# dvrp0/Monsoon

Measured on NVIDIA B200. Metric: env_steps_per_sec, higher is better.
Workload: dtype u8

## Files before the change

### monsoon_b200/csrc/sbw_core.cuh

```cuda
#pragma once
#include "sb_defs.h"
#include "sbw_warp.cuh"

#define WEF_OWNER 1
#define WEF_STRUCT 2
#define WEF_FIXED 4
#define WEF_SINGLE 8
#define WEF_RPLAY 16
#define WEF_ONB 32

struct __align__(8) WCard { u8 card; i8 cost; u8 flags; i8 link; u16 wn; i16 xstr; };
struct __align__(8) WMem { i8 b005; u8 pos, card, fl; i16 strength; u8 st[5]; i8 parent; u8 pad[4]; };
struct WPly {
  i16 base, max_mana, mana;
  i8 front_line;
  u8 replacable, leftmost, n_hand, n_deck, faction;
  u8 pad[4];
  WCard hand[8];
  WCard deck[24];
};
struct __align__(16) WG {
  i16 e_str[MAXE];
  i16 e_dmg[MAXE];
  u32 e_st[MAXE];
  u8 e_card[MAXE], e_fl[MAXE], e_pos[MAXE], e_mid[MAXE], e_plen[MAXE];
  __align__(8) u8 e_path[MAXE][MAXPATH];
  __align__(8) i8 board[24];
  WPly pl[2];
  u32 seed_lo, seed_hi;
  u32 occ, own1, strc;
  u16 turn, draw, steps;
  u8 local_order, current_order, phase, err, done;
  i8 player_sign;
  u8 hist_n, hist_card[4], hist_owner[4];
  u8 n_ent, n_trig, resolving, depth, n_mem, n_obj, maybe_badobs;
  u8 trig[MAXTRIG];
  __align__(8) WMem mem[NMEM];
  u32 lm[SB_MASK_WORDS];
  i8 scr[24];
  i8 tn_ids[24];
  u8 remap[MAXE];
  __align__(8) double scr_d[DECK_W];
  double feat[SB_N_FEATURES];
  const DCard* cards;
  const double* wt;
};

#define WERR(wg, code) do { if (!(wg)->err) (wg)->err = (code); } while (0)
SBW_FI const DCard& WCARD(const WG* wg, int card) { const DCard* c = wg->cards; W_SHARED(c); return c[card]; }
SBW_FI int wpt_x(int pt) { return pt >= 20 ? -1 : (pt & 3); }
SBW_FI int wpt_y(int pt) { return pt == PT_BASE_REMOTE ? -1 : pt == PT_BASE_LOCAL ? 5 : (pt >> 2); }
SBW_FI bool w_valid_xy(int x, int y) { return (unsigned)x <= 3u && (unsigned)y <= 4u; }
SBW_FI int w_owner(const WG* wg, int id) { return wg->e_fl[id] & WEF_OWNER; }
SBW_FI bool w_is_struct(const WG* wg, int id) { return (wg->e_fl[id] & WEF_STRUCT) != 0; }
SBW_FI int w_st(const WG* wg, int id, int s) { return (int)((wg->e_st[id] >> (SB_ST_BITS * s)) & 63u); }
SBW_FI int w_ex(const WG* wg, int id) { return wg->e_pos[id] & 3; }
SBW_FI int w_ey(const WG* wg, int id) { return wg->e_pos[id] >> 2; }

SBW_FI void w_philox(u32 c0, u32 c1, u32 c2, u32 c3, u32 k0, u32 k1, u32& o0, u32& o1) {
#pragma unroll
  for (int r = 0; r < 10; r++) {
    u32 h0 = w_mulhi(0xD2511F53u, c0), l0 = 0xD2511F53u * c0;
    u32 h1 = w_mulhi(0xCD9E8D57u, c2), l1 = 0xCD9E8D57u * c2;
    u32 n0 = h1 ^ c1 ^ k0, n2 = h0 ^ c3 ^ k1;
    c0 = n0; c1 = l1; c2 = n2; c3 = l0;
    k0 += 0x9E3779B9u; k1 += 0xBB67AE85u;
  }
  o0 = c0; o1 = c1;
}
SBW_NI int w_rng_below(WG* wg, int n) {
  W_SHARED(wg);
  if (n <= 0) { WERR(wg, SB_ERR_EMPTY_CHOICE); return 0; }
  u32 w0, w1;
  w_philox(wg->draw, wg->turn, 0, 0, wg->seed_lo, wg->seed_hi, w0, w1);
  wg->draw++;
  return (int)w_mulhi(w0, (u32)n);
}
SBW_NI double w_rng_random(WG* wg) {
  W_SHARED(wg);
  u32 w0, w1;
  w_philox(wg->draw, wg->turn, 0, 0, wg->seed_lo, wg->seed_hi, w0, w1);
  wg->draw++;
  return d_mul(d_add(d_mul((double)(w0 >> 5), 67108864.0), (double)(w1 >> 6)), 0x1.0p-53);
}
SBW_FI u32 w_agent_pick(u32 seed_lo, u32 seed_hi, u32 step, u32 n) {
  u32 w0, w1;
  w_philox(step, 0, 0xA6E7u, 0, seed_lo, seed_hi, w0, w1);
  return w_mulhi(w0, n);
}
SBW void w_shuffle(WG* wg, i8* a, int n) {
#pragma unroll 1
  for (int i = n - 1; i > 0; i--) {
    int j = w_rng_below(wg, i + 1);
    i8 t = a[i]; a[i] = a[j]; a[j] = t;
  }
}

SBW_FI int w_opponent_of(const WG* wg, int order) { return order == 0 ? 1 - wg->local_order : wg->local_order; }
SBW_FI int w_at_xy(const WG* wg, int x, int y) { return w_valid_xy(x, y) ? wg->board[y * 4 + x] : -1; }
SBW_FI int w_at_pt(const WG* wg, int pt) { return (unsigned)pt < 20u ? wg->board[pt] : -1; }
SBW_FI void w_set_xy(WG* wg, int x, int y, int id) {
  const int t = y * 4 + x;
  const u32 b = 1u << t;
  const int prev = wg->board[t];
  if (prev >= 0 && prev != id) wg->e_fl[prev] &= (u8)~WEF_ONB;
  wg->board[t] = (i8)id;
  if (id >= 0) {
    const u8 fl = wg->e_fl[id] | WEF_ONB;
    wg->e_fl[id] = fl;
    wg->e_pos[id] = (u8)t;
    wg->occ |= b;
    wg->own1 = (fl & WEF_OWNER) ? (wg->own1 | b) : (wg->own1 & ~b);
    wg->strc = (fl & WEF_STRUCT) ? (wg->strc | b) : (wg->strc & ~b);
  } else {
    wg->occ &= ~b;
  }
}
SBW_FI void w_clear_at(WG* wg, int id) {
  const int t = wg->e_pos[id];
  const int victim = wg->board[t];
  if (victim >= 0) wg->e_fl[victim] &= (u8)~WEF_ONB;
  wg->board[t] = -1;
  wg->occ &= ~(1u << t);
}
SBW_FI int w_next_tile(u32& m, bool ascending) {
  int t = ascending ? w_ffs(m) - 1 : 31 - w_clz(m);
  m &= ~(1u << t);
  return t;
}
SBW_FI void w_calc_front_line(WG* wg, int order) {
  const bool local = order == wg->local_order;
// ... 270 lines not shown
  if (!w_is_struct(wg, id)) {
    wg->e_plen[id] = 0;
    if (WCARD(wg, wg->e_card[id]).trigger == TR_ON_DEATH) { w_push_trigger(wg, id, has_source); w_pop_trigger(wg); }
  }
  w_calc_front_line(wg, w_opponent_of(wg, wg->current_order));
}
SBW_NI int w_deal_damage(WG* wg, int id, int amount, int pending, int has_source) {
  W_SHARED(wg);
  const int s0 = wg->e_str[id];
  if (s0 - amount < 0) amount = s0;
  wg->e_dmg[id] = (i16)amount;
  const int s1 = s0 - amount;
  wg->e_str[id] = (i16)s1;
  if (!pending && s1 <= 0) w_destroy(wg, id, has_source);
  else if (!w_is_struct(wg, id) && s1 > 0 && WCARD(wg, wg->e_card[id]).trigger == TR_AFTER_SURVIVING) {
    w_push_trigger(wg, id, has_source);
    w_pop_trigger(wg);
  }
  return amount;
}
SBW_FI int w_deal_damage_pt(WG* wg, int pt, int amount, int has_source) {
  if (pt == PT_BASE_LOCAL) return w_player_damage(wg, wg->local_order, amount);
  if (pt == PT_BASE_REMOTE) return w_player_damage(wg, 1 - wg->local_order, amount);
  int id = w_at_pt(wg, pt);
  if (id < 0) { WERR(wg, SB_ERR_NONE_TARGET); return 0; }
  return w_deal_damage(wg, id, amount, 0, has_source);
}

SBW_FI u8 w_enc_xy(int x, int y) { return (u8)((y + 1) * 4 + x); }
SBW_NI void w_set_path(WG* wg, int id, int on_play, int extra_movement) {
  W_SHARED(wg);
  u64 dest = 0;
  int nd = 0;
  int px = w_ex(wg, id), py = w_ey(wg, id);
  int confused_cached = w_st(wg, id, SB_ST_CONFUSED);
  const int fl = wg->e_fl[id];
  const int owner = fl & WEF_OWNER;
  const bool is_local = owner == wg->local_order;
  int steps = on_play ? WCARD(wg, wg->e_card[id]).movement + extra_movement : 1;
  if (steps > MAXPATH) { WERR(wg, SB_ERR_OVERFLOW); steps = MAXPATH; }
  const u32 mine = owner ? wg->own1 : ~wg->own1;
#pragma unroll 1
  for (int i = 0; i < steps; i++) {
    int dx = px, dy = py + (is_local ? -1 : 1);
    if (confused_cached > 0) {
      int delta;
      if (px == 0) { w_rng_below(wg, 1); delta = 1; }
      else if (px == 3) { w_rng_below(wg, 1); delta = -1; }
      else delta = w_rng_below(wg, 2) == 0 ? -1 : 1;
      dx = px + delta; dy = py;
      confused_cached--;
    } else if (on_play && !(fl & WEF_FIXED) && dy != (is_local ? -1 : 5)) {
      const u32 occ = wg->occ;
      const bool ahead_free_or_own = !w_valid_xy(dx, dy) || !((occ >> (dy * 4 + dx)) & 1u) || ((mine >> (dy * 4 + dx)) & 1u);
      if (ahead_free_or_own) {
        const int t = py * 4 + px;
        bool left_ok = px > 0 && w_valid_xy(px - 1, py) && ((occ & ~mine) >> (t - 1) & 1u);
        bool right_ok = px < 3 && w_valid_xy(px + 1, py) && ((occ & ~mine) >> (t + 1) & 1u);
        const u8 lenc = w_enc_xy(px - 1, py), renc = w_enc_xy(px + 1, py);
#pragma unroll 1
        for (int k = 0; k < nd; k++) {
          const u8 d = (u8)(dest >> (8 * k));
          if (d == lenc) left_ok = false;
          if (d == renc) right_ok = false;
        }
        if (px <= 1) { if (right_ok) { dx = px + 1; dy = py; } else if (left_ok) { dx = px - 1; dy = py; } }
        else { if (left_ok) { dx = px - 1; dy = py; } else if (right_ok) { dx = px + 1; dy = py; } }
      }
    }
    dest |= (u64)w_enc_xy(dx, dy) << (8 * nd);
    nd++;
    px = dx; py = dy;
  }
  *reinterpret_cast<u64*>(wg->e_path[id]) = dest;
  wg->e_plen[id] = (u8)nd;
}
SBW_FI void w_set_path_step(WG* wg, int id) {
  if (w_st(wg, id, SB_ST_CONFUSED)) { w_set_path(wg, id, 0, 0); return; }
  const int t = wg->e_pos[id];
  const bool is_local = w_owner(wg, id) == wg->local_order;
  wg->e_path[id][0] = (u8)(t + 4 + (is_local ? -4 : 4));
  wg->e_plen[id] = 1;
}
SBW_NI void w_unit_move(WG* wg, int id) {
  W_SHARED(wg);
  if (wg->depth > MAXDEPTH) { WERR(wg, SB_ERR_DEPTH); return; }
  wg->depth++;
  const int trig = WCARD(wg, wg->e_card[id]).trigger;
  const u8 current_id = (u8)(wg->e_mid[id] + 1);
  wg->e_mid[id] = current_id;
  if (wg->phase == PH_TURN_START) {
    if (w_st(wg, id, SB_ST_POISONED)) w_deal_damage(wg, id, 1, 0, 0);
    else if (w_st(wg, id, SB_ST_VITALIZED)) wv_heal(wg, id, 1);
    if (w_st(wg, id, SB_ST_FROZEN)) { w_st_remove(wg, id, SB_ST_FROZEN); wg->depth--; return; }
  }
  if (wg->e_plen[id] == 0) { wg->depth--; return; }
  if (trig == TR_BEFORE_MOVING && !w_st(wg, id, SB_ST_DISABLED)) w_ability(wg, id, PT_NONE, 1);
  if (w_st(wg, id, SB_ST_FROZEN)) { wg->depth--; return; }
  const int np = wg->e_plen[id];
  const u64 path = *reinterpret_cast<const u64*>(wg->e_path[id]);
#pragma unroll 1
  for (int i = 0; i < np; i++) {
    const int enc = (int)((path >> (8 * i)) & 0xFFu);
    const int dx = enc & 3, dy = (enc >> 2) - 1;
    const int owner = w_owner(wg, id);
    if (dy < 0 || dy > 4) {
      if (trig == TR_BEFORE_ATTACKING && !w_st(wg, id, SB_ST_DISABLED)) w_ability(wg, id, -2, 1);
      const int target = dy < 0 ? 1 - wg->local_order : wg->local_order;
      w_player_damage(wg, target, wg->e_str[id]);
      if (wg->pl[target].base > 0) w_destroy(wg, id, 0);
      wg->depth--;
      return;
    }
    int tid = w_at_xy(wg, dx, dy);
    bool attacked = false;
    if (tid >= 0 && w_owner(wg, tid) == owner && dx == w_ex(wg, id)) { wg->depth--; return; }
    if (tid >= 0 && (w_st(wg, id, SB_ST_CONFUSED) || w_owner(wg, tid) != owner)) {
      if (trig == TR_BEFORE_ATTACKING && !w_st(wg, id, SB_ST_DISABLED)) w_ability(wg, id, dy * 4 + dx, 1);
      tid = w_at_xy(wg, dx, dy);
      if (tid >= 0) {
        const int tstr = wg->e_str[tid];
        const int t_pending = !w_is_struct(wg, tid) && WCARD(wg, wg->e_card[tid]).trigger == TR_ON_DEATH && !w_st(wg, tid, SB_ST_DISABLED);
        const int l_pending = trig == TR_ON_DEATH && !w_st(wg, id, SB_ST_DISABLED);
        w_deal_damage(wg, tid, wg->e_str[id], t_pending, 0);
        w_deal_damage(wg, id, tstr, l_pending, 0);
        if (wg->e_str[tid] <= 0 && t_pending) w_destroy(wg, tid, 0);
        if (wg->e_str[id] <= 0 && l_pending) w_destroy(wg, id, 0);
        attacked = true;
      }
    }
    if (current_id != wg->e_mid[id]) { wg->depth--; return; }
    if (w_at_xy(wg, dx, dy) < 0 && wg->e_str[id] > 0) {
      w_clear_at(wg, id);
      w_set_xy(wg, dx, dy, id);
      WPly& p = wg->pl[w_owner(wg, id)];
      if (p.front_line > dy) p.front_line = (i8)(dy > 1 ? dy : 1);
      if (attacked && trig == TR_AFTER_ATTACKING && !w_st(wg, id, SB_ST_DISABLED)) w_ability(wg, id, PT_NONE, 1);
      if (w_st(wg, id, SB_ST_CONFUSED)) w_st_remove(wg, id, SB_ST_CONFUSED);
    }
  }
  wg->depth--;
}
SBW_FI void w_unit_play(WG* wg, int id, int x, int y) {
  wg->e_fl[id] |= WEF_RPLAY;
  w_set_xy(wg, x, y, id);
  w_set_path(wg, id, 1, 0);
  if (WCARD(wg, wg->e_card[id]).trigger == TR_ON_PLAY) w_ability(wg, id, PT_NONE, 1);
  w_unit_move(wg, id);
  wg->e_fl[id] &= (u8)~WEF_RPLAY;
}
SBW_NI void w_struct_play(WG* wg, int id, int x, int y) {
  W_SHARED(wg);
  w_set_xy(wg, x, y, id);
  if (WCARD(wg, wg->e_card[id]).trigger == TR_ON_PLAY) w_ability(wg, id, PT_NONE, 1);
}
SBW_FI void w_gain_speed(WG* wg, int id, int amount) { w_set_path(wg, id, (wg->e_fl[id] & WEF_RPLAY) != 0, amount); }
SBW_NI void wv_command(WG* wg, int id) {
  W_SHARED(wg);
  const u8 cache = wg->e_fl[id] & WEF_FIXED;
  wg->e_fl[id] |= WEF_FIXED;
  w_set_path_step(wg, id);
  w_unit_move(wg, id);
  wg->e_fl[id] = (u8)((wg->e_fl[id] & ~WEF_FIXED) | cache);
}
SBW_NI void wv_convert(WG* wg, int id) {
  W_SHARED(wg);
  const int o = w_opponent_of(wg, w_owner(wg, id));
  wg->e_fl[id] = (u8)((wg->e_fl[id] & ~WEF_OWNER) | (o ? WEF_OWNER : 0));
  const int t = wg->e_pos[id];
  if (wg->board[t] == id) {
    const u32 b = 1u << t;
    wg->own1 = o ? (wg->own1 | b) : (wg->own1 & ~b);
  }
  w_set_path(wg, id, (wg->e_fl[id] & WEF_RPLAY) != 0, 0);
}
SBW_NI void wv_push(WG* wg, int id, int fx, int fy) {
  W_SHARED(wg);
  int dx = 0, dy = 0;
  const int ex = w_ex(wg, id), ey = w_ey(wg, id);
  if (fy < ey) dy = 1; else if (fy > ey) dy = -1; else if (fx < ex) dx = 1; else if (fx > ex) dx = -1;
  if (dx || dy) {
#pragma unroll 1
    for (;;) {
      const int nx = w_ex(wg, id) + dx, ny = w_ey(wg, id) + dy;
      if (!w_valid_xy(nx, ny)) break;
      if (wg->board[ny * 4 + nx] >= 0) return;
      w_clear_at(wg, id);
      w_set_xy(wg, nx, ny, id);
    }
  }
  WPly& p = wg->pl[w_owner(wg, id)];
  const int y = w_ey(wg, id);
  if (p.front_line > y) p.front_line = (i8)(y > 1 ? y : 1);
}
SBW_NI void wv_force_attack(WG* wg, int id, int tx, int ty) {
  W_SHARED(wg);
  const int ex = w_ex(wg, id), ey = w_ey(wg, id);
  if ((tx != ex && ty != ey) || w_at_xy(wg, tx, ty) < 0) return;
  u64 dest = 0;
  int nd = 0;
  const bool vertical = (tx == ex);
  const int fixed = vertical ? ex : ey, start = vertical ? ey : ex, end = vertical ? ty : tx;
  const int delta = end > start ? 1 : -1;
#pragma unroll 1
  for (int i = start + delta; i != end + delta; i += delta) {
    const int x = vertical ? fixed : i, y = vertical ? i : fixed;
    if (i != end && w_at_xy(wg, x, y) >= 0) return;
    dest |= (u64)w_enc_xy(x, y) << (8 * nd);
    nd++;
  }
  if (nd > 0) {
    *reinterpret_cast<u64*>(wg->e_path[id]) = dest;
    wg->e_plen[id] = (u8)nd;
    w_unit_move(wg, id);
  }
}
SBW_NI void wv_teleport(WG* wg, int id, int dx, int dy) {
  W_SHARED(wg);
  if (w_at_xy(wg, dx, dy) < 0) {
    w_clear_at(wg, id);
    w_set_xy(wg, dx, dy, id);
    WPly& p = wg->pl[w_owner(wg, id)];
    if (p.front_line > dy) p.front_line = (i8)(dy > 1 ? dy : 1);
    w_set_path(wg, id, (wg->e_fl[id] & WEF_RPLAY) != 0, 0);
  }
// ... 342 lines not shown
```

### monsoon_b200/csrc/sbw_kernels.cu

```cuda
#include <cuda_runtime.h>
#include <stdint.h>
#include <stdlib.h>
#include "sbw_agent.cuh"
#include "sbw_launch.h"

#define W_SLOT_BYTES ((int)((sizeof(WG) + sizeof(SbState) + 15) & ~15u))

__device__ __forceinline__ void kw_stage_cards(DCard* s_cards, const DCard* cards) {
  const u32* src = reinterpret_cast<const u32*>(cards);
  u32* dst = reinterpret_cast<u32*>(s_cards);
  for (int i = threadIdx.x; i < (int)(SBC_COUNT * sizeof(DCard) / 4); i += blockDim.x) dst[i] = __ldg(src + i);
  __syncthreads();
}
__device__ __forceinline__ WG* kw_slot(unsigned char* dyn, int warp, int slot_bytes) { return reinterpret_cast<WG*>(dyn + (size_t)warp * slot_bytes); }
__device__ __forceinline__ SbState* kw_image(WG* wg) { return reinterpret_cast<SbState*>(reinterpret_cast<unsigned char*>(wg) + sizeof(WG)); }
__device__ __forceinline__ void kw_load_record(SbState* img, const u8* states, int gi) {
  const int lane = threadIdx.x & 31;
  reinterpret_cast<uint4*>(img)[lane] = __ldg(reinterpret_cast<const uint4*>(states + (size_t)gi * SB_STATE_BYTES) + lane);
  __syncwarp();
}
__device__ __forceinline__ void kw_store_record(u8* states, int gi, const SbState* img) {
  const int lane = threadIdx.x & 31;
  __syncwarp();
  reinterpret_cast<uint4*>(states + (size_t)gi * SB_STATE_BYTES)[lane] = reinterpret_cast<const uint4*>(img)[lane];
}
__device__ __forceinline__ int kw_next_game(int* queue, int fallback) {
  if (!queue) return fallback;
  int gi = 0;
  if ((threadIdx.x & 31) == 0) gi = atomicAdd(queue, 1);
  return __shfl_sync(0xFFFFFFFFu, gi, 0);
}

template <int WPC, int MINB, int SYNC>
__global__ void __launch_bounds__(WPC * 32, MINB) kw_rollout_random(int n, u8* states, int max_steps, int* steps_out, unsigned long long* chain,
                                                                     const DCard* cards, const double* wt, int* queue) {
  __shared__ DCard s_cards[SBC_COUNT];
  extern __shared__ __align__(16) unsigned char s_dyn[];
  kw_stage_cards(s_cards, cards);
  const int warp = threadIdx.x >> 5, lane = threadIdx.x & 31;
  WG* wg = kw_slot(s_dyn, warp, W_SLOT_BYTES);
  SbState* img = kw_image(wg);
  wg->cards = s_cards; wg->wt = wt;
  const bool digest = chain != nullptr;
  int gi = blockIdx.x * WPC + warp;
  if (SYNC == 0) {
#pragma unroll 1
    for (;;) {
      gi = kw_next_game(queue, gi);
      if (gi >= n) break;
      kw_load_record(img, states, gi);
      w_unpack(wg, img);
      unsigned long long ch = digest ? chain[gi] : 0ull;
      int k = 0;
      bool alive = !(wg->done & SB_DONE) && !wg->err && max_steps > 0;
#pragma unroll 1
      while (alive) {
        w_game_step(wg, w_pick_action(wg));
        w_end_of_step(wg);
        if (digest) { w_pack(wg, img); __syncwarp(); ch = (ch ^ w_digest_state(img)) * 0x100000001B3ull; }
        k++;
        alive = !(wg->done & SB_DONE) && !wg->err && k < max_steps;
      }
      w_pack(wg, img);
      kw_store_record(states, gi, img);
      if (lane == 0) {
        if (steps_out) steps_out[gi] = k;
        if (digest) chain[gi] = ch;
      }
      if (!queue) break;
      __syncwarp();
    }
  } else {
    bool has_game = false, alive = false, at_pass = false, dry = false;
    unsigned long long ch = 0ull;
    int k = 0;
    bool first = true;
#pragma unroll 1
    for (;;) {
      if (!alive && !dry) {
        if (has_game) {
          w_pack(wg, img);
          kw_store_record(states, gi, img);
          if (lane == 0) { if (steps_out) steps_out[gi] = k; if (digest) chain[gi] = ch; }
          __syncwarp();
          has_game = false;
        }
        if (queue) gi = kw_next_game(queue, gi); else if (!first) gi = n;
        first = false;
        if (gi < n) {
          has_game = true;
          kw_load_record(img, states, gi);
          w_unpack(wg, img);
          ch = digest ? chain[gi] : 0ull;
          k = 0; at_pass = false;
          alive = !(wg->done & SB_DONE) && !wg->err && max_steps > 0;
        } else dry = true;
      }
      if (!__syncthreads_or(alive)) break;
#pragma unroll 1
      for (;;) {
        int a = -1;
        if (alive && !at_pass) {
          a = w_pick_action(wg);
          if (a == SB_ACTION_PASS) { at_pass = true; a = -1; }
        }
        if (SYNC == 2) {
          if (a < 0) { __syncthreads(); break; }
        } else if (!__syncthreads_or(a >= 0)) break;
        if (a >= 0) {
          w_game_step(wg, a);
          w_end_of_step(wg);
          if (digest) { w_pack(wg, img); __syncwarp(); ch = (ch ^ w_digest_state(img)) * 0x100000001B3ull; }
          k++;
          alive = !(wg->done & SB_DONE) && !wg->err && k < max_steps;
        }
      }
      if (alive && at_pass) {
        w_game_step(wg, SB_ACTION_PASS);
        w_end_of_step(wg);
        if (digest) { w_pack(wg, img); __syncwarp(); ch = (ch ^ w_digest_state(img)) * 0x100000001B3ull; }
        k++;
        at_pass = false;
        alive = !(wg->done & SB_DONE) && !wg->err && k < max_steps;
      }
    }
    if (has_game) {
      w_pack(wg, img);
      kw_store_record(states, gi, img);
      if (lane == 0) { if (steps_out) steps_out[gi] = k; if (digest) chain[gi] = ch; }
    }
  }
}

template <int WPC>
__global__ void __launch_bounds__(WPC * 32) kw_step(int n, u8* states, const u8* actions, i8* reward, u8* done, u8* err, u32* next_masks,
                                                    const DCard* cards, const double* wt) {
  __shared__ DCard s_cards[SBC_COUNT];
  extern __shared__ __align__(16) unsigned char s_dyn[];
  kw_stage_cards(s_cards, cards);
  const int warp = threadIdx.x >> 5, lane = threadIdx.x & 31;
  WG* wg = kw_slot(s_dyn, warp, W_SLOT_BYTES);
  SbState* img = kw_image(wg);
  wg->cards = s_cards; wg->wt = wt;
#pragma unroll 1
  for (int gi = blockIdx.x * WPC + warp; gi < n; gi += gridDim.x * WPC) {
    kw_load_record(img, states, gi);
    w_unpack(wg, img);
    w_game_step(wg, actions[gi]);
    w_pack(wg, img);
    kw_store_record(states, gi, img);
    if (lane == 0) {
      if (reward) reward[gi] = (wg->done & SB_REWARD) ? 1 : 0;
      if (done) done[gi] = (wg->done & SB_DONE) ? 1 : 0;
      if (err) err[gi] = img->err;
    }
    if (next_masks) {
      w_legal_mask(wg);
      if (lane < SB_MASK_WORDS) next_masks[(size_t)gi * SB_MASK_WORDS + lane] = wg->lm[lane];
    }
    __syncwarp();
  }
}

template <int WPC, int MODE>
__global__ void __launch_bounds__(WPC * 32, 2048 / (WPC * 32)) kw_stream(int n, const u8* states, void* out, u8* err, const DCard* cards) {
  __shared__ DCard s_cards[SBC_COUNT];
  __shared__ __align__(16) SbState s_img[WPC];
  __shared__ __align__(16) int s_out[MODE == 1 ? WPC * SB_OBS_INTS : (MODE == 2 ? WPC * 2 * SB_N_FEATURES : 4)];
  kw_stage_cards(s_cards, cards);
  const int warp = threadIdx.x >> 5, lane = threadIdx.x & 31;
  const int stride = gridDim.x * WPC;
  int gi = blockIdx.x * WPC + warp;
  uint4 nxt = make_uint4(0, 0, 0, 0);
  if (gi < n) nxt = __ldg(reinterpret_cast<const uint4*>(states + (size_t)gi * SB_STATE_BYTES) + lane);
#pragma unroll 1
  for (; gi < n; gi += stride) {
    const uint4 cur = nxt;
    if (gi + stride < n) nxt = __ldg(reinterpret_cast<const uint4*>(states + (size_t)(gi + stride) * SB_STATE_BYTES) + lane);
    reinterpret_cast<uint4*>(&s_img[warp])[lane] = cur;
    __syncwarp();
    if (MODE == 0) {
      u32 m[SB_MASK_WORDS];
      w_legal_mask_packed(&s_img[warp], s_cards, m);
      const u32 v = lane == 0 ? m[0] : lane == 1 ? m[1] : lane == 2 ? m[2] : lane == 3 ? m[3] : m[4];
      if (lane < SB_MASK_WORDS) reinterpret_cast<u32*>(out)[(size_t)gi * SB_MASK_WORDS + lane] = v;
    } else if (MODE == 1) {
      int* ob = s_out + warp * SB_OBS_INTS;
      const int e = w_observe_packed(&s_img[warp], s_cards, ob);
      uint4* dst = reinterpret_cast<uint4*>(reinterpret_cast<int*>(out) + (size_t)gi * SB_OBS_INTS);
      const uint4* src = reinterpret_cast<const uint4*>(ob);
#pragma unroll
      for (int i = lane; i < SB_OBS_INTS / 4; i += 32) dst[i] = src[i];
      if (err && lane == 0) err[gi] = (u8)e;
    } else {
      double* f = reinterpret_cast<double*>(s_out) + warp * SB_N_FEATURES;
      const int e = w_features_packed(&s_img[warp], s_cards, f);
      __syncwarp();
      if (lane < SB_N_FEATURES) reinterpret_cast<double*>(out)[(size_t)gi * SB_N_FEATURES + lane] = f[lane];
      if (err && lane == 0) err[gi] = (u8)e;
    }
    __syncwarp();
  }
}

template <int WPC, int MODE>
__global__ void __launch_bounds__(WPC * 32) kw_query(int n, u8* states, void* out, u8* err, const DCard* cards, const double* wt) {
  __shared__ DCard s_cards[SBC_COUNT];
  extern __shared__ __align__(16) unsigned char s_dyn[];
  kw_stage_cards(s_cards, cards);
  const int warp = threadIdx.x >> 5, lane = threadIdx.x & 31;
  WG* wg = kw_slot(s_dyn, warp, W_SLOT_BYTES);
  SbState* img = kw_image(wg);
  wg->cards = s_cards; wg->wt = wt;
#pragma unroll 1
  for (int gi = blockIdx.x * WPC + warp; gi < n; gi += gridDim.x * WPC) {
    kw_load_record(img, states, gi);
    w_unpack(wg, img);
    if (MODE == 0) {
      w_legal_mask(wg);
      if (lane < SB_MASK_WORDS) reinterpret_cast<u32*>(out)[(size_t)gi * SB_MASK_WORDS + lane] = wg->lm[lane];
    } else if (MODE == 1) {
      const int e = w_observe(wg, reinterpret_cast<int*>(out) + (size_t)gi * SB_OBS_INTS);
      if (err && lane == 0) err[gi] = (u8)e;
    } else if (MODE == 2) {
      w_scan_badobs(wg);
      const int e = w_features(wg, wg->feat);
      if (lane < SB_N_FEATURES) reinterpret_cast<double*>(out)[(size_t)gi * SB_N_FEATURES + lane] = wg->feat[lane];
      if (err && lane == 0) err[gi] = (u8)e;
    } else {
      const int a = w_expert_action(wg);
      if (lane == 0) {
        reinterpret_cast<u8*>(out)[gi] = (u8)a;
        SbState* rec = reinterpret_cast<SbState*>(states + (size_t)gi * SB_STATE_BYTES);
        rec->draw = wg->draw;
        rec->err = wg->err;
      }
    }
    __syncwarp();
  }
}

#define W_HSLOT_BYTES ((int)((2 * sizeof(WG) + sizeof(SbState) + 2 * SB_N_FEATURES * sizeof(double) + 15) & ~15u))
__device__ __forceinline__ WG* kw_hfork(WG* base) { return base + 1; }
__device__ __forceinline__ SbState* kw_himage(WG* base) { return reinterpret_cast<SbState*>(base + 2); }
__device__ __forceinline__ double* kw_hweights(WG* base) { return reinterpret_cast<double*>(reinterpret_cast<unsigned char*>(base + 2) + sizeof(SbState)); }

template <int WPC>
__global__ void __launch_bounds__(WPC * 32) kw_select_action(int n, const u8* states, const double* weights, u8* actions, double* scores,
                                                             const DCard* cards, const double* wt) {
  __shared__ DCard s_cards[SBC_COUNT];
  extern __shared__ __align__(16) unsigned char s_dyn[];
  kw_stage_cards(s_cards, cards);
  const int warp = threadIdx.x >> 5, lane = threadIdx.x & 31;
  WG* base = kw_slot(s_dyn, warp, W_HSLOT_BYTES);
  WG* work = kw_hfork(base);
  SbState* img = kw_himage(base);
  double* w = kw_hweights(base);
  base->cards = s_cards; base->wt = wt; work->cards = s_cards; work->wt = wt;
#pragma unroll 1
  for (int gi = blockIdx.x * WPC + warp; gi < n; gi += gridDim.x * WPC) {
    kw_load_record(img, states, gi);
    w_unpack(base, img);
    w_scan_badobs(base);
    if (lane < SB_N_FEATURES) w[lane] = weights[(size_t)gi * SB_N_FEATURES + lane];
    if (scores) for (int a = lane; a < SB_N_ACTIONS; a += 32) scores[(size_t)gi * SB_N_ACTIONS + a] = __longlong_as_double(0x7FF8000000000000ll);
    __syncwarp();
    const int a = w_decide(base, work, w, scores ? scores + (size_t)gi * SB_N_ACTIONS : nullptr, false);
    if (lane == 0) actions[gi] = (u8)a;
    __syncwarp();
  }
}

template <int WPC, int MINB>
__global__ void __launch_bounds__(WPC * 32, MINB) kw_rollout_heuristic(int n, u8* states, const double* w_first, const double* w_second, const int* idx_first,
                                                                        const int* idx_second, int max_steps, i8* result, int* steps_out,
                                                                        const DCard* cards, const double* wt, int* queue) {
  __shared__ DCard s_cards[SBC_COUNT];
  extern __shared__ __align__(16) unsigned char s_dyn[];
  kw_stage_cards(s_cards, cards);
  const int warp = threadIdx.x >> 5, lane = threadIdx.x & 31;
  WG* base = kw_slot(s_dyn, warp, W_HSLOT_BYTES);
  WG* work = kw_hfork(base);
  SbState* img = kw_himage(base);
  double* wf = kw_hweights(base);
  double* ws = wf + SB_N_FEATURES;
  base->cards = s_cards; base->wt = wt; work->cards = s_cards; work->wt = wt;
  int gi = blockIdx.x * WPC + warp;
#pragma unroll 1
  for (;;) {
    gi = kw_next_game(queue, gi);
    if (gi >= n) break;
    kw_load_record(img, states, gi);
    w_unpack(base, img);
    w_scan_badobs(base);
    if (lane < SB_N_FEATURES) {
      if (w_first) wf[lane] = w_first[(size_t)(idx_first ? idx_first[gi] : gi) * SB_N_FEATURES + lane];
      if (w_second) ws[lane] = w_second[(size_t)(idx_second ? idx_second[gi] : gi) * SB_N_FEATURES + lane];
    }
    __syncwarp();
    int k = 0, res = -1;
#pragma unroll 1
    for (;;) {
      if (k >= max_steps || base->pl[0].base < 0 || base->pl[1].base < 0) break;
      const bool first_to_move = base->player_sign == 1;
      if (first_to_move ? w_first != nullptr : w_second != nullptr) w_decide(base, work, first_to_move ? wf : ws, nullptr, true);
      else {
        const int a = w_expert_action(base);
        w_game_step(base, a);
        w_end_of_step(base);
      }
      k++;
      if (base->err) { res = -2; break; }
    }
    if (res != -2) {
      const bool l0 = base->pl[0].base < 0, l1 = base->pl[1].base < 0;
      res = (l1 && !l0) ? 0 : (l0 && !l1) ? 1 : -1;
    }
    w_pack(base, img);
    kw_store_record(states, gi, img);
    if (lane == 0) {
      if (result) result[gi] = (i8)res;
      if (steps_out) steps_out[gi] = k;
    }
    if (!queue) break;
    __syncwarp();
  }
}

static inline int grid_for(int n, int per) { return (n + per - 1) / per; }
static int g_carveout = -1;
template <class K> static cudaError_t set_smem(K kernel, int bytes) {
  cudaError_t e = cudaFuncSetAttribute(kernel, cudaFuncAttributeMaxDynamicSharedMemorySize, bytes);
  if (e != cudaSuccess || g_carveout < 0) return e;
  return cudaFuncSetAttribute(kernel, cudaFuncAttributePreferredSharedMemoryCarveout, g_carveout);
}
#define W_TRY(x) do { cudaError_t e_ = (x); if (e_ != cudaSuccess) return e_; } while (0)

int sbw_wg_bytes(void) { return (int)sizeof(WG); }

cudaError_t sbw_init(void) {
  { const char* e = getenv("SBW_CARVEOUT"); if (e) g_carveout = atoi(e); }
  W_TRY((set_smem(kw_rollout_random<4, 8, 0>, 4 * W_SLOT_BYTES)));
  W_TRY((set_smem(kw_rollout_random<8, 4, 0>, 8 * W_SLOT_BYTES)));
  W_TRY((set_smem(kw_rollout_random<8, 8, 0>, 8 * W_SLOT_BYTES)));
  W_TRY((set_smem(kw_rollout_random<8, 4, 1>, 8 * W_SLOT_BYTES)));
  W_TRY((set_smem(kw_rollout_random<16, 2, 1>, 16 * W_SLOT_BYTES)));
  W_TRY((set_smem(kw_rollout_random<32, 1, 1>, 32 * W_SLOT_BYTES)));
  W_TRY((set_smem(kw_rollout_random<32, 2, 1>, 32 * W_SLOT_BYTES)));
  W_TRY((set_smem(kw_rollout_random<28, 1, 1>, 28 * W_SLOT_BYTES)));
  W_TRY((set_smem(kw_rollout_random<14, 2, 1>, 14 * W_SLOT_BYTES)));
  W_TRY((set_smem(kw_rollout_random<32, 1, 2>, 32 * W_SLOT_BYTES)));
  W_TRY((set_smem(kw_rollout_random<16, 2, 2>, 16 * W_SLOT_BYTES)));
  W_TRY(set_smem(kw_step<8>, 8 * W_SLOT_BYTES));
  W_TRY(set_smem(kw_query<8, 3>, 8 * W_SLOT_BYTES));
  W_TRY(set_smem(kw_select_action<4>, 4 * W_HSLOT_BYTES));
  W_TRY(set_smem(kw_rollout_heuristic<4, 8>, 4 * W_HSLOT_BYTES));
  W_TRY(set_smem(kw_rollout_heuristic<4, 9>, 4 * W_HSLOT_BYTES));
  return cudaSuccess;
}

void sbw_rollout_random(const SbwCtx* c, int n, uint8_t* states, int max_steps, int32_t* steps, uint64_t* chain, int shape, int grid_override,
                        cudaStream_t st) {
  static const int WPCS[11] = {8, 4, 8, 8, 16, 32, 32, 28, 14, 32, 16}, PER_SM[11] = {4, 8, 8, 4, 2, 1, 2, 1, 2, 1, 2};
  if (shape < 0 || shape > 10) shape = 0;
  const int wpc = WPCS[shape], per_sm = PER_SM[shape];
  const int resident = c->sm_count * per_sm;
  const int full = grid_for(n, wpc);
  int* q = nullptr;
  int grid = full;
  if (grid_override > 0 || full > resident) {
    q = c->d_queue;
    cudaMemsetAsync(q, 0, sizeof(int), st);
    grid = grid_override > 0 ? grid_override : resident;
  }
  unsigned long long* ch = (unsigned long long*)chain;
#define RR(W, B, S) kw_rollout_random<W, B, S><<<grid, W * 32, W * W_SLOT_BYTES, st>>>(n, states, max_steps, steps, ch, c->d_cards, c->d_wt, q)
  switch (shape) {
    case 0: RR(8, 4, 0); break;
    case 1: RR(4, 8, 0); break;
    case 2: RR(8, 8, 0); break;
    case 3: RR(8, 4, 1); break;
    case 4: RR(16, 2, 1); break;
    case 5: RR(32, 1, 1); break;
    case 6: RR(32, 2, 1); break;
    case 7: RR(28, 1, 1); break;
    case 8: RR(14, 2, 1); break;
    case 9: RR(32, 1, 2); break;
    default: RR(16, 2, 2); break;
  }
#undef RR
}
static inline int query_grid(const SbwCtx* c, int n, int wpc) {
  const int full = grid_for(n, wpc), cap = c->sm_count * 32;
  return full < cap ? full : cap;
}
void sbw_step(const SbwCtx* c, int n, uint8_t* states, const uint8_t* actions, int8_t* reward, uint8_t* done, uint8_t* err, uint32_t* next_masks,
              cudaStream_t st) {
  kw_step<8><<<query_grid(c, n, 8), 256, 8 * W_SLOT_BYTES, st>>>(n, states, actions, (i8*)reward, done, err, next_masks, c->d_cards, c->d_wt);
}
void sbw_legal_mask(const SbwCtx* c, int n, const uint8_t* states, uint32_t* masks, cudaStream_t st) {
  const int full = grid_for(n, 8), cap = c->sm_count * 8;
  kw_stream<8, 0><<<full < cap ? full : cap, 256, 0, st>>>(n, states, masks, nullptr, c->d_cards);
}
void sbw_observe(const SbwCtx* c, int n, const uint8_t* states, int32_t* obs, uint8_t* err, cudaStream_t st) {
  const int full = grid_for(n, 8), cap = c->sm_count * 8;
  kw_stream<8, 1><<<full < cap ? full : cap, 256, 0, st>>>(n, states, obs, err, c->d_cards);
}
void sbw_features(const SbwCtx* c, int n, const uint8_t* states, double* feat, uint8_t* err, cudaStream_t st) {
  const int full = grid_for(n, 8), cap = c->sm_count * 8;
  kw_stream<8, 2><<<full < cap ? full : cap, 256, 0, st>>>(n, states, feat, err, c->d_cards);
}
void sbw_expert_action(const SbwCtx* c, int n, uint8_t* states, uint8_t* actions, cudaStream_t st) {
  kw_query<8, 3><<<query_grid(c, n, 8), 256, 8 * W_SLOT_BYTES, st>>>(n, states, actions, nullptr, c->d_cards, c->d_wt);
}
void sbw_select_action(const SbwCtx* c, int n, const uint8_t* states, const double* weights, uint8_t* actions, double* scores, cudaStream_t st) {
  kw_select_action<4><<<query_grid(c, n, 4), 128, 4 * W_HSLOT_BYTES, st>>>(n, states, weights, actions, scores, c->d_cards, c->d_wt);
}
void sbw_rollout_heuristic(const SbwCtx* c, int n, uint8_t* states, const double* w_first, const double* w_second, const int32_t* idx_first,
                           const int32_t* idx_second, int max_steps, int8_t* result, int32_t* steps, int shape, int grid_override, cudaStream_t st) {
  const int wpc = 4, per_sm = shape == 1 ? 9 : 8;
  const int resident = c->sm_count * per_sm, full = grid_for(n, wpc);
  int* q = nullptr;
  int grid = full;
  if (grid_override > 0 || full > resident) {
    q = c->d_queue + 1;
    cudaMemsetAsync(q, 0, sizeof(int), st);
    grid = grid_override > 0 ? grid_override : resident;
  }
  if (shape == 1)
    kw_rollout_heuristic<4, 9><<<grid, 128, 4 * W_HSLOT_BYTES, st>>>(n, states, w_first, w_second, idx_first, idx_second, max_steps, (i8*)result, steps,
                                                                    c->d_cards, c->d_wt, q);
  else
    kw_rollout_heuristic<4, 8><<<grid, 128, 4 * W_HSLOT_BYTES, st>>>(n, states, w_first, w_second, idx_first, idx_second, max_steps, (i8*)result, steps,
                                                                   c->d_cards, c->d_wt, q);
}
```

### monsoon_b200/csrc/sbw_warp.cuh

```cuda
#pragma once
#include <stdint.h>

#if defined(__CUDA_ARCH__)
#define SBW __device__
#define SBW_NI __device__ __noinline__
#define SBW_FI __device__ __forceinline__
#define W_FULL 0xFFFFFFFFu
#define FOR_LANES(l) { const int l = (int)(threadIdx.x & 31u);
#define END_LANES } __syncwarp();
template <class T> struct LV { T v; };
#define LVAL(x, l) ((x).v)
#define W_SHARED(p) __builtin_assume(__isShared(p))
#else
#include <math.h>
#include <string.h>
#define SBW static
#define SBW_NI static __attribute__((noinline))
#define SBW_FI static inline
#define FOR_LANES(l) for (int l = 0; l < 32; l++) {
#define END_LANES }
template <class T> struct LV { T v[32]; };
#define LVAL(x, l) ((x).v[l])
#define W_SHARED(p) ((void)0)
#ifndef __align__
#define __align__(n) __attribute__((aligned(n)))
#endif
#endif

typedef signed char i8;
typedef unsigned char u8;
typedef short i16;
typedef unsigned short u16;
typedef unsigned int u32;
typedef unsigned long long u64;

#if defined(__CUDA_ARCH__)
SBW_FI u32 w_mulhi(u32 a, u32 b) { return __umulhi(a, b); }
SBW_FI int w_popc(u32 x) { return __popc(x); }
SBW_FI int w_ffs(u32 x) { return __ffs(x); }
SBW_FI int w_clz(u32 x) { return __clz(x); }
SBW_FI u32 w_brev(u32 x) { return __brev(x); }
SBW_FI double d_add(double a, double b) { return __dadd_rn(a, b); }
SBW_FI double d_sub(double a, double b) { return __dsub_rn(a, b); }
SBW_FI double d_mul(double a, double b) { return __dmul_rn(a, b); }
SBW_FI double d_fma(double a, double b, double c) { return __fma_rn(a, b, c); }
SBW_FI double d_hilo(u32 hi, u32 lo) { return __hiloint2double((int)hi, (int)lo); }
#else
SBW_FI u32 w_mulhi(u32 a, u32 b) { return (u32)(((u64)a * (u64)b) >> 32); }
SBW_FI int w_popc(u32 x) { return __builtin_popcount(x); }
SBW_FI int w_ffs(u32 x) { return __builtin_ffs((int)x); }
SBW_FI int w_clz(u32 x) { return x ? __builtin_clz(x) : 32; }
SBW_FI u32 w_brev(u32 x) { u32 r = 0; for (int i = 0; i < 32; i++) r |= ((x >> i) & 1u) << (31 - i); return r; }
SBW_FI double d_add(double a, double b) { return a + b; }
SBW_FI double d_sub(double a, double b) { return a - b; }
SBW_FI double d_mul(double a, double b) { return a * b; }
SBW_FI double d_fma(double a, double b, double c) { return fma(a, b, c); }
SBW_FI double d_hilo(u32 hi, u32 lo) { u64 b = ((u64)hi << 32) | lo; double d; memcpy(&d, &b, 8); return d; }
#endif
#if defined(__CUDA_ARCH__)
SBW_NI double d_div(double a, double b) { return __ddiv_rn(a, b); }
#else
SBW_NI double d_div(double a, double b) { return a / b; }
#endif

template <class F> SBW_FI u32 w_ballot(F f) {
#if defined(__CUDA_ARCH__)
  return __ballot_sync(W_FULL, f((int)(threadIdx.x & 31u)));
#else
  u32 m = 0;
  for (int l = 0; l < 32; l++) m |= (f(l) ? 1u : 0u) << l;
  return m;
#endif
}
template <class F> SBW_FI u32 w_or(F f) {
#if defined(__CUDA_ARCH__)
  return __reduce_or_sync(W_FULL, (u32)f((int)(threadIdx.x & 31u)));
#else
  u32 m = 0;
  for (int l = 0; l < 32; l++) m |= (u32)f(l);
  return m;
#endif
}
template <class F> SBW_FI int w_sum(F f) {
#if defined(__CUDA_ARCH__)
  return __reduce_add_sync(W_FULL, (int)f((int)(threadIdx.x & 31u)));
#else
  int s = 0;
  for (int l = 0; l < 32; l++) s += (int)f(l);
  return s;
#endif
}
template <class F> SBW_FI int w_min(F f) {
#if defined(__CUDA_ARCH__)
  return __reduce_min_sync(W_FULL, (int)f((int)(threadIdx.x & 31u)));
#else
  int s = 0x7FFFFFFF;
// ... 37 lines not shown
```

Baseline: 83.98 million.

## Spill unit-move locals to explicit per-warp frame stack in shared memory

Keeps w_unit_move's live state (path, trigger, move id, loop index, target info) in an explicit frame record pushed onto a per-warp stack instead of in registers across recursive calls. The record is reloaded after each nested call. For rollout kernels with at most 32 warps per SM the stack sits in shared memory, otherwise in local memory. The aim is to cut register pressure and ABI spill cost in the recursive non-inlined call chain, at the price of extra shared-memory traffic and a larger shared allocation that may reduce occupancy.

```diff
diff --git a/monsoon_b200/csrc/sbw_core.cuh b/monsoon_b200/csrc/sbw_core.cuh
--- a/monsoon_b200/csrc/sbw_core.cuh
+++ b/monsoon_b200/csrc/sbw_core.cuh
@@ -44,9 +44,40 @@
   double feat[SB_N_FEATURES];
   const DCard* cards;
   const double* wt;
+  u8* fsp;
+  u8* fse;
 };
 
 #define WERR(wg, code) do { if (!(wg)->err) (wg)->err = (code); } while (0)
+
+struct WMoveRec {
+  u64 path;
+  i16 tstr;
+  u8 id, trig, cur, np, i, tid, fl;
+  u8 pad[5];
+};
+#define W_FRAME_BYTES ((MAXDEPTH + 1) * (int)sizeof(WMoveRec))
+static_assert(sizeof(WMoveRec) == 24 && W_FRAME_BYTES % 8 == 0, "frame stack layout");
+#if !defined(__CUDA_ARCH__)
+static __align__(8) u8 w_host_frames[W_FRAME_BYTES];
+static int w_frame_high_water = 0;
+#endif
+template <class R> SBW_FI R* w_push(WG* wg) {
+#if !defined(__CUDA_ARCH__)
+  if (!wg->fsp) { wg->fsp = w_host_frames; wg->fse = w_host_frames + W_FRAME_BYTES; }
+#endif
+  u8* p = wg->fsp;
+#if !defined(__CUDA_ARCH__)
+  assert(p + sizeof(R) <= wg->fse);
+  const int used = (int)(p + sizeof(R) - (wg->fse - W_FRAME_BYTES));
+  if (used > w_frame_high_water) w_frame_high_water = used;
+#endif
+  if (p + sizeof(R) > wg->fse) { WERR(wg, SB_ERR_DEPTH); return nullptr; }
+  wg->fsp = p + sizeof(R);
+  return reinterpret_cast<R*>(p);
+}
+template <class R> SBW_FI R* w_top(const WG* wg) { return reinterpret_cast<R*>(wg->fsp - sizeof(R)); }
+template <class R> SBW_FI void w_pop(WG* wg) { wg->fsp -= sizeof(R); }
 SBW_FI const DCard& WCARD(const WG* wg, int card) { const DCard* c = wg->cards; W_SHARED(c); return c[card]; }
 SBW_FI int wpt_x(int pt) { return pt >= 20 ? -1 : (pt & 3); }
 SBW_FI int wpt_y(int pt) { return pt == PT_BASE_REMOTE ? -1 : pt == PT_BASE_LOCAL ? 5 : (pt >> 2); }
@@ -483,65 +514,76 @@
   wg->e_path[id][0] = (u8)(t + 4 + (is_local ? -4 : 4));
   wg->e_plen[id] = 1;
 }
+#define WM_RELOAD() (f = w_top<WMoveRec>(wg), id = f->id)
 SBW_NI void w_unit_move(WG* wg, int id) {
   W_SHARED(wg);
   if (wg->depth > MAXDEPTH) { WERR(wg, SB_ERR_DEPTH); return; }
   wg->depth++;
-  const int trig = WCARD(wg, wg->e_card[id]).trigger;
-  const u8 current_id = (u8)(wg->e_mid[id] + 1);
-  wg->e_mid[id] = current_id;
+  WMoveRec* f = w_push<WMoveRec>(wg);
+  if (!f) { wg->depth--; return; }
+  f->id = (u8)id;
+  f->trig = (u8)WCARD(wg, wg->e_card[id]).trigger;
+  f->cur = (u8)(wg->e_mid[id] + 1);
+  wg->e_mid[id] = f->cur;
   if (wg->phase == PH_TURN_START) {
-    if (w_st(wg, id, SB_ST_POISONED)) w_deal_damage(wg, id, 1, 0, 0);
+    if (w_st(wg, id, SB_ST_POISONED)) { w_deal_damage(wg, id, 1, 0, 0); WM_RELOAD(); }
     else if (w_st(wg, id, SB_ST_VITALIZED)) wv_heal(wg, id, 1);
-    if (w_st(wg, id, SB_ST_FROZEN)) { w_st_remove(wg, id, SB_ST_FROZEN); wg->depth--; return; }
-  }
-  if (wg->e_plen[id] == 0) { wg->depth--; return; }
-  if (trig == TR_BEFORE_MOVING && !w_st(wg, id, SB_ST_DISABLED)) w_ability(wg, id, PT_NONE, 1);
-  if (w_st(wg, id, SB_ST_FROZEN)) { wg->depth--; return; }
-  const int np = wg->e_plen[id];
-  const u64 path = *reinterpret_cast<const u64*>(wg->e_path[id]);
-#pragma unroll 1
-  for (int i = 0; i < np; i++) {
-    const int enc = (int)((path >> (8 * i)) & 0xFFu);
-    const int dx = enc & 3, dy = (enc >> 2) - 1;
+    if (w_st(wg, id, SB_ST_FROZEN)) { w_st_remove(wg, id, SB_ST_FROZEN); goto out; }
+  }
+  if (wg->e_plen[id] == 0) goto out;
+  if (f->trig == TR_BEFORE_MOVING && !w_st(wg, id, SB_ST_DISABLED)) { w_ability(wg, id, PT_NONE, 1); WM_RELOAD(); }
+  if (w_st(wg, id, SB_ST_FROZEN)) goto out;
+  f->np = wg->e_plen[id];
+  f->path = *reinterpret_cast<const u64*>(wg->e_path[id]);
+#pragma unroll 1
+  for (f->i = 0; f->i < f->np; f->i++) {
+    int enc = (int)((f->path >> (8 * f->i)) & 0xFFu);
+    int dx = enc & 3, dy = (enc >> 2) - 1;
     const int owner = w_owner(wg, id);
     if (dy < 0 || dy > 4) {
-      if (trig == TR_BEFORE_ATTACKING && !w_st(wg, id, SB_ST_DISABLED)) w_ability(wg, id, -2, 1);
+      if (f->trig == TR_BEFORE_ATTACKING && !w_st(wg, id, SB_ST_DISABLED)) { w_ability(wg, id, -2, 1); WM_RELOAD(); dy = (int)((f->path >> (8 * f->i + 2)) & 0x3Fu) - 1; }
       const int target = dy < 0 ? 1 - wg->local_order : wg->local_order;
       w_player_damage(wg, target, wg->e_str[id]);
       if (wg->pl[target].base > 0) w_destroy(wg, id, 0);
-      wg->depth--;
-      return;
+      goto out;
     }
     int tid = w_at_xy(wg, dx, dy);
-    bool attacked = false;
-    if (tid >= 0 && w_owner(wg, tid) == owner && dx == w_ex(wg, id)) { wg->depth--; return; }
+    f->fl = 0;
+    if (tid >= 0 && w_owner(wg, tid) == owner && dx == w_ex(wg, id)) goto out;
     if (tid >= 0 && (w_st(wg, id, SB_ST_CONFUSED) || w_owner(wg, tid) != owner)) {
-      if (trig == TR_BEFORE_ATTACKING && !w_st(wg, id, SB_ST_DISABLED)) w_ability(wg, id, dy * 4 + dx, 1);
-      tid = w_at_xy(wg, dx, dy);
+      if (f->trig == TR_BEFORE_ATTACKING && !w_st(wg, id, SB_ST_DISABLED)) { w_ability(wg, id, dy * 4 + dx, 1); WM_RELOAD(); }
+      enc = (int)((f->path >> (8 * f->i)) & 0xFFu);
+      tid = w_at_xy(wg, enc & 3, (enc >> 2) - 1);
       if (tid >= 0) {
-        const int tstr = wg->e_str[tid];
-        const int t_pending = !w_is_struct(wg, tid) && WCARD(wg, wg->e_card[tid]).trigger == TR_ON_DEATH && !w_st(wg, tid, SB_ST_DISABLED);
-        const int l_pending = trig == TR_ON_DEATH && !w_st(wg, id, SB_ST_DISABLED);
-        w_deal_damage(wg, tid, wg->e_str[id], t_pending, 0);
-        w_deal_damage(wg, id, tstr, l_pending, 0);
-        if (wg->e_str[tid] <= 0 && t_pending) w_destroy(wg, tid, 0);
-        if (wg->e_str[id] <= 0 && l_pending) w_destroy(wg, id, 0);
-        attacked = true;
+        f->tstr = wg->e_str[tid];
+        f->tid = (u8)tid;
+        f->fl = (u8)(1 | ((!w_is_struct(wg, tid) && WCARD(wg, wg->e_card[tid]).trigger == TR_ON_DEATH && !w_st(wg, tid, SB_ST_DISABLED)) ? 2 : 0) |
+                     ((f->trig == TR_ON_DEATH && !w_st(wg, id, SB_ST_DISABLED)) ? 4 : 0));
+        w_deal_damage(wg, tid, wg->e_str[id], (f->fl >> 1) & 1, 0);
+        WM_RELOAD();
+        w_deal_damage(wg, id, f->tstr, (f->fl >> 2) & 1, 0);
+        WM_RELOAD();
+        if (wg->e_str[f->tid] <= 0 && (f->fl & 2)) { w_destroy(wg, f->tid, 0); WM_RELOAD(); }
+        if (wg->e_str[id] <= 0 && (f->fl & 4)) { w_destroy(wg, id, 0); WM_RELOAD(); }
       }
     }
-    if (current_id != wg->e_mid[id]) { wg->depth--; return; }
+    if (f->cur != wg->e_mid[id]) goto out;
+    enc = (int)((f->path >> (8 * f->i)) & 0xFFu);
+    dx = enc & 3; dy = (enc >> 2) - 1;
     if (w_at_xy(wg, dx, dy) < 0 && wg->e_str[id] > 0) {
       w_clear_at(wg, id);
       w_set_xy(wg, dx, dy, id);
       WPly& p = wg->pl[w_owner(wg, id)];
       if (p.front_line > dy) p.front_line = (i8)(dy > 1 ? dy : 1);
-      if (attacked && trig == TR_AFTER_ATTACKING && !w_st(wg, id, SB_ST_DISABLED)) w_ability(wg, id, PT_NONE, 1);
+      if ((f->fl & 1) && f->trig == TR_AFTER_ATTACKING && !w_st(wg, id, SB_ST_DISABLED)) { w_ability(wg, id, PT_NONE, 1); WM_RELOAD(); }
       if (w_st(wg, id, SB_ST_CONFUSED)) w_st_remove(wg, id, SB_ST_CONFUSED);
     }
   }
+out:
+  w_pop<WMoveRec>(wg);
   wg->depth--;
 }
+#undef WM_RELOAD
 SBW_FI void w_unit_play(WG* wg, int id, int x, int y) {
   wg->e_fl[id] |= WEF_RPLAY;
   w_set_xy(wg, x, y, id);
diff --git a/monsoon_b200/csrc/sbw_kernels.cu b/monsoon_b200/csrc/sbw_kernels.cu
--- a/monsoon_b200/csrc/sbw_kernels.cu
+++ b/monsoon_b200/csrc/sbw_kernels.cu
@@ -24,6 +24,9 @@
   __syncwarp();
   reinterpret_cast<uint4*>(states + (size_t)gi * SB_STATE_BYTES)[lane] = reinterpret_cast<const uint4*>(img)[lane];
 }
+__host__ __device__ constexpr bool kw_frames_shared(int wpc, int minb) { return wpc * minb <= 32; }
+__host__ __device__ constexpr int kw_rr_smem(int wpc, int minb) { return wpc * (W_SLOT_BYTES + (kw_frames_shared(wpc, minb) ? W_FRAME_BYTES : 0)); }
+__device__ __forceinline__ void kw_frames(WG* wg, u8* stack) { wg->fsp = stack; wg->fse = stack + W_FRAME_BYTES; }
 __device__ __forceinline__ int kw_next_game(int* queue, int fallback) {
   if (!queue) return fallback;
   int gi = 0;
@@ -41,6 +44,8 @@
   WG* wg = kw_slot(s_dyn, warp, W_SLOT_BYTES);
   SbState* img = kw_image(wg);
   wg->cards = s_cards; wg->wt = wt;
+  __align__(8) u8 l_frames[kw_frames_shared(WPC, MINB) ? 8 : W_FRAME_BYTES];
+  kw_frames(wg, kw_frames_shared(WPC, MINB) ? s_dyn + WPC * W_SLOT_BYTES + warp * W_FRAME_BYTES : l_frames);
   const bool digest = chain != nullptr;
   int gi = blockIdx.x * WPC + warp;
   if (SYNC == 0) {
@@ -142,6 +147,8 @@
   WG* wg = kw_slot(s_dyn, warp, W_SLOT_BYTES);
   SbState* img = kw_image(wg);
   wg->cards = s_cards; wg->wt = wt;
+  __align__(8) u8 l_frames[W_FRAME_BYTES];
+  kw_frames(wg, l_frames);
 #pragma unroll 1
   for (int gi = blockIdx.x * WPC + warp; gi < n; gi += gridDim.x * WPC) {
     kw_load_record(img, states, gi);
@@ -212,6 +219,8 @@
   WG* wg = kw_slot(s_dyn, warp, W_SLOT_BYTES);
   SbState* img = kw_image(wg);
   wg->cards = s_cards; wg->wt = wt;
+  __align__(8) u8 l_frames[W_FRAME_BYTES];
+  kw_frames(wg, l_frames);
 #pragma unroll 1
   for (int gi = blockIdx.x * WPC + warp; gi < n; gi += gridDim.x * WPC) {
     kw_load_record(img, states, gi);
@@ -257,6 +266,9 @@
   SbState* img = kw_himage(base);
   double* w = kw_hweights(base);
   base->cards = s_cards; base->wt = wt; work->cards = s_cards; work->wt = wt;
+  __align__(8) u8 l_frames[W_FRAME_BYTES];
+  kw_frames(base, l_frames);
+  kw_frames(work, l_frames);
 #pragma unroll 1
   for (int gi = blockIdx.x * WPC + warp; gi < n; gi += gridDim.x * WPC) {
     kw_load_record(img, states, gi);
@@ -285,6 +297,9 @@
   double* wf = kw_hweights(base);
   double* ws = wf + SB_N_FEATURES;
   base->cards = s_cards; base->wt = wt; work->cards = s_cards; work->wt = wt;
+  __align__(8) u8 l_frames[W_FRAME_BYTES];
+  kw_frames(base, l_frames);
+  kw_frames(work, l_frames);
   int gi = blockIdx.x * WPC + warp;
 #pragma unroll 1
   for (;;) {
@@ -340,17 +355,17 @@
 
 cudaError_t sbw_init(void) {
   { const char* e = getenv("SBW_CARVEOUT"); if (e) g_carveout = atoi(e); }
-  W_TRY((set_smem(kw_rollout_random<4, 8, 0>, 4 * W_SLOT_BYTES)));
-  W_TRY((set_smem(kw_rollout_random<8, 4, 0>, 8 * W_SLOT_BYTES)));
-  W_TRY((set_smem(kw_rollout_random<8, 8, 0>, 8 * W_SLOT_BYTES)));
-  W_TRY((set_smem(kw_rollout_random<8, 4, 1>, 8 * W_SLOT_BYTES)));
-  W_TRY((set_smem(kw_rollout_random<16, 2, 1>, 16 * W_SLOT_BYTES)));
-  W_TRY((set_smem(kw_rollout_random<32, 1, 1>, 32 * W_SLOT_BYTES)));
-  W_TRY((set_smem(kw_rollout_random<32, 2, 1>, 32 * W_SLOT_BYTES)));
-  W_TRY((set_smem(kw_rollout_random<28, 1, 1>, 28 * W_SLOT_BYTES)));
-  W_TRY((set_smem(kw_rollout_random<14, 2, 1>, 14 * W_SLOT_BYTES)));
-  W_TRY((set_smem(kw_rollout_random<32, 1, 2>, 32 * W_SLOT_BYTES)));
-  W_TRY((set_smem(kw_rollout_random<16, 2, 2>, 16 * W_SLOT_BYTES)));
+  W_TRY((set_smem(kw_rollout_random<4, 8, 0>, kw_rr_smem(4, 8))));
+  W_TRY((set_smem(kw_rollout_random<8, 4, 0>, kw_rr_smem(8, 4))));
+  W_TRY((set_smem(kw_rollout_random<8, 8, 0>, kw_rr_smem(8, 8))));
+  W_TRY((set_smem(kw_rollout_random<8, 4, 1>, kw_rr_smem(8, 4))));
+  W_TRY((set_smem(kw_rollout_random<16, 2, 1>, kw_rr_smem(16, 2))));
+  W_TRY((set_smem(kw_rollout_random<32, 1, 1>, kw_rr_smem(32, 1))));
+  W_TRY((set_smem(kw_rollout_random<32, 2, 1>, kw_rr_smem(32, 2))));
+  W_TRY((set_smem(kw_rollout_random<28, 1, 1>, kw_rr_smem(28, 1))));
+  W_TRY((set_smem(kw_rollout_random<14, 2, 1>, kw_rr_smem(14, 2))));
+  W_TRY((set_smem(kw_rollout_random<32, 1, 2>, kw_rr_smem(32, 1))));
+  W_TRY((set_smem(kw_rollout_random<16, 2, 2>, kw_rr_smem(16, 2))));
   W_TRY(set_smem(kw_step<8>, 8 * W_SLOT_BYTES));
   W_TRY(set_smem(kw_query<8, 3>, 8 * W_SLOT_BYTES));
   W_TRY(set_smem(kw_select_action<4>, 4 * W_HSLOT_BYTES));
@@ -374,7 +389,7 @@
     grid = grid_override > 0 ? grid_override : resident;
   }
   unsigned long long* ch = (unsigned long long*)chain;
-#define RR(W, B, S) kw_rollout_random<W, B, S><<<grid, W * 32, W * W_SLOT_BYTES, st>>>(n, states, max_steps, steps, ch, c->d_cards, c->d_wt, q)
+#define RR(W, B, S) kw_rollout_random<W, B, S><<<grid, W * 32, kw_rr_smem(W, B), st>>>(n, states, max_steps, steps, ch, c->d_cards, c->d_wt, q)
   switch (shape) {
     case 0: RR(8, 4, 0); break;
     case 1: RR(4, 8, 0); break;
diff --git a/monsoon_b200/csrc/sbw_warp.cuh b/monsoon_b200/csrc/sbw_warp.cuh
--- a/monsoon_b200/csrc/sbw_warp.cuh
+++ b/monsoon_b200/csrc/sbw_warp.cuh
@@ -12,6 +12,7 @@
 #define LVAL(x, l) ((x).v)
 #define W_SHARED(p) __builtin_assume(__isShared(p))
 #else
+#include <assert.h>
 #include <math.h>
 #include <string.h>
 #define SBW static
```

After: 78.03 million, median of 6. 0.929x the previous value.
